# yuguangnudt/VEC_VAD

Hardware: AMD Instinct MI355X
Metric: spatio-temporal cubes/sec (train step) (higher is better)
Workload: dtype f32

## Files before the change

include/vecvad_hip.h:

```cpp
#ifndef VECVAD_HIP_H
#define VECVAD_HIP_H

#include <stddef.h>
#include <stdint.h>

#ifdef __cplusplus
extern "C" {
#endif

typedef void* vv_stream;

enum vv_status {
  VV_OK = 0,
  VV_ERR_BAD_ARG = 1,
  VV_ERR_LAUNCH = 2,
  VV_ERR_UNSUPPORTED = 3
};

enum vv_in_mode {
  VV_IN_PLAIN = 0,
  VV_IN_ACT = 1,
  VV_IN_POOL = 2,
  VV_IN_CAT = 3,
  VV_IN_CUBE = 4,
  VV_IN_BNBWD = 5
};

enum vv_conv_kind {
  VV_CONV3 = 0,
  VV_CONVT_FWD = 1,
  VV_CONVT_DGRAD = 2
};

typedef struct vv_view {
  float* ptr;
  int64_t gstride;
  int32_t cstride;
  int32_t coff;
} vv_view;

#define VV_CONV_BF16 1
#define VV_CONV_SRC_BF16 2
#define VV_CONV_OUT_BF16 8
#define VV_CONV_ALLSRC_BF16 16
#define VV_CONV_RELU 32
#define VV_CONV_NO_GEMM16 64
#define VV_CONV_NO_RING 128
typedef struct vv_conv_params {
  int32_t kind;
  int32_t in_mode;
  int32_t G, B;
  int32_t H, W;
  int32_t Cin;
  int32_t CinP;
  int32_t Cout;
  vv_view src0;
  const float* a;
  const float* b;
  int64_t ab_gstride;
  vv_view src1;
  int32_t csplit;
  int32_t pad0;
  const int32_t* chmap;
  const float* w;
  int64_t w_gstride;
  const float* bias;
  int64_t bias_gstride;
  vv_view out;
  float* stats;
  const float* bn_z; int64_t bn_z_gstride;
  const float* bn_a; const float* bn_b; const float* bn_mean; const float* bn_invstd; int64_t bn_gstride;
  float* bn_partial;
  vv_view out1;
  int32_t osplit;
  int32_t pad1;
} vv_conv_params;

int vv_conv_mfma(const vv_conv_params* p, vv_stream stream);
int vv_conv_ntiles(int32_t B, int32_t H, int32_t W);
int vv_conv_ntiles2(int32_t B, int32_t H, int32_t W, int32_t kind, int32_t flags);
int vv_convt_dgrad_ntiles(int32_t B, int32_t H, int32_t W, int32_t flags);

typedef struct vv_wgrad_params {
  int32_t kind;
  int32_t in_mode;
  int32_t G, B, H, W;
  int32_t Cin, CinP, Cout;
  int32_t ksplit;
  vv_view src0; const float* a; const float* b; int64_t ab_gstride;
  vv_view src1; int32_t csplit;
  int32_t pad0;
  const int32_t* chmap;
  vv_view dy;
  float* partial;
  int64_t partial_gstride;
  vv_view dy_z;
  const float* dy_bn; int64_t dy_bn_gstride;
} vv_wgrad_params;

int vv_wgrad_mfma(const vv_wgrad_params* p, vv_stream stream);
int vv_wgrad_ntiles(int32_t kind, int32_t B, int32_t H, int32_t W);

#define VV_WGRAD_X_BF16 2
#define VV_WGRAD_DY_BF16 1
int vv_wgrad_bf16(const vv_wgrad_params* p, vv_stream stream);
int vv_wgrad_bf16_plan(int32_t kind, int32_t B, int32_t H, int32_t W, int32_t CinP, int32_t Cout, int32_t* ntiles, int32_t* nblocks,
                       int32_t* kw);

int vv_wgrad_reduce(int32_t kind, int32_t G, int32_t Cin, int32_t CinP, int32_t Cout, int32_t nslab_per_tile,
                    const float* partial, int64_t partial_gstride, float* grad, int64_t grad_gstride,
                    vv_stream stream);
typedef struct vv_reduce_entry {
  int32_t kind, Cin, Cout, NCO, nslab, block_start;
  int64_t part_off, grad_off, grad_gstride;
} vv_reduce_entry;
int vv_wgrad_reduce_grouped(const vv_reduce_entry* table_dev, int32_t nentries, int32_t total_blocks, int32_t G, const float* partial,
                            int64_t partial_gstride, float* grads, vv_stream stream);

#define VV_PACK_BF16 4
typedef struct vv_pack_entry {
  int64_t src_off;
  int64_t dst_off;
  int32_t mode, K, KP, N;
} vv_pack_entry;
int vv_pack_weights(const vv_pack_entry* table_dev, int32_t nentries, int32_t G, const float* params,
                    int64_t params_gstride, float* packed, int64_t packed_gstride, int32_t max_elems,
                    vv_stream stream);

int vv_conv_wino(const vv_conv_params* p, vv_stream stream);
int vv_wino_ntiles(int32_t B, int32_t H);
// ... 285 lines not shown
```

vec_vad_amd/_lib.py:

```python
import ctypes as C
import os

import torch

HERE = os.path.dirname(os.path.abspath(__file__))
LIB_PATH = os.environ.get('VV_LIB_PATH') or os.path.join(HERE, 'csrc', 'libvecvad_hip.so')

c_i32, c_i64, c_f32, c_f64, c_vp = C.c_int32, C.c_int64, C.c_float, C.c_double, C.c_void_p

IN_PLAIN, IN_ACT, IN_POOL, IN_CAT, IN_CUBE, IN_BNBWD = 0, 1, 2, 3, 4, 5
BNBWD_TAB_ROWS = 7
CONV3, CONVT_FWD, CONVT_DGRAD = 0, 1, 2
CONV_BF16 = 1
CONV_SRC_BF16 = 2
PACK_BF16 = 4
BNBWD_DZ_BF16 = 1
BNBWD_PARTIALS_PER_CUBE = 2
BNBWD_DA_BF16 = 4
CONV_OUT_BF16 = 8
CONV_ALLSRC_BF16 = 16
CONV_RELU = 32
CONV_NO_GEMM16 = 64
CONV_NO_RING = 128
BNBWD_Y_BF16 = 8
BNBWD_PARTIALS_PER_TILE = 16
BNBWD_PARTIALS_PER_CTILE = 32
BNBWD_PARTIALS_PER_TILE44 = 64
BNBWD_PARTIALS_PER_TTILE = 128
WGRAD_X_BF16 = 2
WGRAD_DY_BF16 = 1


class View(C.Structure):
    _fields_ = [('ptr', c_vp), ('gstride', c_i64), ('cstride', c_i32), ('coff', c_i32)]


class ConvParams(C.Structure):
    _fields_ = [('kind', c_i32), ('in_mode', c_i32), ('G', c_i32), ('B', c_i32), ('H', c_i32), ('W', c_i32),
                ('Cin', c_i32), ('CinP', c_i32), ('Cout', c_i32),
                ('src0', View), ('a', c_vp), ('b', c_vp), ('ab_gstride', c_i64),
                ('src1', View), ('csplit', c_i32), ('pad0', c_i32), ('chmap', c_vp),
                ('w', c_vp), ('w_gstride', c_i64), ('bias', c_vp), ('bias_gstride', c_i64),
                ('out', View), ('stats', c_vp),
                ('bn_z', c_vp), ('bn_z_gstride', c_i64), ('bn_a', c_vp), ('bn_b', c_vp), ('bn_mean', c_vp), ('bn_invstd', c_vp),
                ('bn_gstride', c_i64), ('bn_partial', c_vp),
                ('out1', View), ('osplit', c_i32), ('pad1', c_i32)]


class WgradParams(C.Structure):
    _fields_ = [('kind', c_i32), ('in_mode', c_i32), ('G', c_i32), ('B', c_i32), ('H', c_i32), ('W', c_i32),
                ('Cin', c_i32), ('CinP', c_i32), ('Cout', c_i32), ('ksplit', c_i32),
                ('src0', View), ('a', c_vp), ('b', c_vp), ('ab_gstride', c_i64),
                ('src1', View), ('csplit', c_i32), ('pad0', c_i32), ('chmap', c_vp),
                ('dy', View), ('partial', c_vp), ('partial_gstride', c_i64),
                ('dy_z', View), ('dy_bn', c_vp), ('dy_bn_gstride', c_i64)]


class PackEntry(C.Structure):
    _fields_ = [('src_off', c_i64), ('dst_off', c_i64), ('mode', c_i32), ('K', c_i32), ('KP', c_i32), ('N', c_i32)]


class ReduceEntry(C.Structure):
    _fields_ = [('kind', c_i32), ('Cin', c_i32), ('Cout', c_i32), ('NCO', c_i32), ('nslab', c_i32), ('block_start', c_i32),
                ('part_off', c_i64), ('grad_off', c_i64), ('grad_gstride', c_i64)]


class FoldEntry(C.Structure):
    _fields_ = [('w_off', c_i64), ('b_off', c_i64), ('g_off', c_i64), ('beta_off', c_i64), ('rm_off', c_i64), ('rv_off', c_i64),
                ('cout', c_i32), ('row', c_i32)]


class BnBwdParams(C.Structure):
    _fields_ = [('G', c_i32), ('B', c_i32), ('H', c_i32), ('W', c_i32), ('C', c_i32), ('flags', c_i32),
                ('y', c_vp), ('y_gstride', c_i64),
                ('a', c_vp), ('b', c_vp), ('mean', c_vp), ('invstd', c_vp), ('ab_gstride', c_i64),
                ('dA', View), ('dpool', c_vp), ('dpool_gstride', c_i64),
                ('dz', c_vp), ('dz_gstride', c_i64), ('partial', c_vp)]


class OutconvParams(C.Structure):
    _fields_ = [('G', c_i32), ('B', c_i32), ('HW', c_i32), ('C', c_i32),
                ('y', c_vp), ('y_gstride', c_i64), ('a', c_vp), ('b', c_vp), ('ab_gstride', c_i64),
                ('w', c_vp), ('bias', c_vp), ('param_gstride', c_i64), ('oc', c_vp),
                ('tgt0', c_vp), ('tgt0_cstride', c_i32), ('pad0', c_i32),
                ('tgt1', c_vp), ('tgt1_cstride', c_i32), ('pad1', c_i32),
                ('tgt_src', c_vp), ('tgt_coff', c_vp), ('out4', c_vp), ('score', c_vp), ('gscale', c_vp),
                ('dout4', c_vp)]


class Conv2dParams(C.Structure):
    _fields_ = [('kind', c_i32), ('R', c_i32), ('stride', c_i32), ('B', c_i32), ('H', c_i32), ('W', c_i32),
                ('Cin', c_i32), ('CinP', c_i32), ('Cout', c_i32), ('CoutP', c_i32), ('src', View), ('w', c_vp),
                ('bias', c_vp), ('slope', c_f32), ('pad0', c_i32), ('out', View)]


_SIGS = {
    'vv_conv2d_mfma': (c_i32, [C.POINTER(Conv2dParams), c_vp]),
    'vv_conv2d_wino': (c_i32, [c_vp, c_i32, c_i32, c_i64, c_vp, c_vp, c_f32, c_vp, c_i32, c_i32, c_i32, c_i32, c_i32, c_i32, c_i32, c_vp]),
    'vv_conv2d_splitk_finish': (c_i32, [c_vp, c_i32, c_i64, c_i32, c_i32, c_vp, c_f32, c_vp, c_i32, c_i32, c_vp]),
    'vv_pack_conv2d': (c_i32, [c_vp, c_vp, c_i32, c_i32, c_i32, c_i32, c_i32, c_i32, c_vp]),
    'vv_conv3x3_n2': (c_i32, [c_vp, c_i32, c_i32, c_i32, c_i32, c_i32, c_vp, c_i32, c_vp, c_f32, c_vp, c_i32, c_i32, c_vp]),
    'vv_deconv4x4_c2': (c_i32, [c_vp, c_i32, c_i32, c_i32, c_i32, c_vp, c_vp, c_f32, c_vp, c_i32, c_i32, c_vp]),
    'vv_upsample4': (c_i32, [c_vp, c_vp, c_i32, c_i32, c_i32, c_i32, c_f32, c_vp]),
    'vv_conv_mfma': (c_i32, [C.POINTER(ConvParams), c_vp]),
    'vv_conv_wino': (c_i32, [C.POINTER(ConvParams), c_vp]),
    'vv_wino_ntiles': (c_i32, [c_i32, c_i32]),
# ... 153 lines not shown
```

vec_vad_amd/csrc/vv_conv.hip:

```cpp
#include "vv_common.h"
#ifndef VV_PD_BF
#define VV_PD_BF 1
#endif

namespace {

template <int KIND, int TH, int TW>
struct Geo {
  static constexpr int HH = KIND == VV_CONV3 ? TH + 2 : (KIND == VV_CONVT_FWD ? TH + 1 : 2 * TH + 1);
  static constexpr int HW = KIND == VV_CONV3 ? TW + 2 : (KIND == VV_CONVT_FWD ? TW + 1 : 2 * TW + 1);
  static constexpr int SP = KIND == VV_CONVT_DGRAD ? 2 : 1;
};

template <int TH, int TW, int NI, int NR, int KIND, int CK, bool BF, int S16, int MR>
__global__ void __launch_bounds__(VV_WG, (MR == 1 && BF) ? 4 : ((BF && KIND == VV_CONVT_DGRAD) ? 1 : ((NR == 1 && KIND != VV_CONVT_FWD && !(BF && NI >= 4)) ? 3 : 2)))
conv_mfma_kernel(const vv_conv_params p, const int NT, const int NN, const int total, const int nper) {
  using G_ = Geo<KIND, TH, TW>;
  constexpr int HH = G_::HH, HW = G_::HW, SP = G_::SP;
  static_assert(!BF || CK % 16 == 0, "bf16 K step = 16 channels");
  constexpr int S = BF ? CK / 2 + ((CK / 8) % 2 ? 8 : 4) : CK + 4;
  constexpr int S4 = S / 4;
  static_assert(S4 % 2 == 1, "odd float4 stride");
  static_assert(TH * TW * NI == 128 * MR, "tile pixels");
  constexpr int TN = NR * 32;
  constexpr int KGC = BF ? CK / 16 : CK / 8;
  constexpr int A4 = NI * HH * HW * S4;
  constexpr int BROWS = 9 * KGC * 2;
  constexpr int B4 = BROWS * TN;
  constexpr int NBT = (B4 + VV_WG - 1) / VV_WG;
  constexpr int ORS = TN + 8, OUT4 = (BF && KIND != VV_CONVT_FWD) ? (128 * MR * ORS * 2 + 15) / 16 : 0;
  constexpr int LDS4 = (A4 + B4) > OUT4 ? (A4 + B4) : OUT4;
  __shared__ float4 lds4[LDS4];
  float* lds = reinterpret_cast<float*>(lds4);
  const v4f* ldsA = reinterpret_cast<const v4f*>(lds4);
  const v4f* ldsB = reinterpret_cast<const v4f*>(lds4) + A4;

  int w = vv_xcd_remap(blockIdx.x, nper);
  if (w >= total) return;
  const int nn = w % NN; w /= NN;
  const int pt = w % NT; w /= NT;
  const int g = w;

  const int tid = threadIdx.x, lane = tid & 63, wave = tid >> 6, half = lane >> 5, l31 = lane & 31;
  const int H = p.H, W = p.W;
  const int tilesX = W / TW, tilesY = H / TH;
  const int tpi = tilesX * tilesY;
  const int img0 = (pt / tpi) * NI;
  const int trem = pt % tpi;
  const int ty0 = (trem / tilesX) * TH, tx0 = (trem % tilesX) * TW;

  const int SH = KIND == VV_CONVT_DGRAD ? 2 * H : H, SW = KIND == VV_CONVT_DGRAD ? 2 * W : W;
  const int oy0 = KIND == VV_CONV3 ? ty0 - 1 : (KIND == VV_CONVT_FWD ? ty0 : 2 * ty0 - 1);
  const int ox0 = KIND == VV_CONV3 ? tx0 - 1 : (KIND == VV_CONVT_FWD ? tx0 : 2 * tx0 - 1);

  const VVSrc s = vv_make_src(p, g, SH, SW);
  const int Cout = p.Cout, CinP = p.CinP, KQ = CinP >> 3;
  const int co0 = nn * TN;
  const float* __restrict__ wg = p.w + (int64_t)g * p.w_gstride;

  int abase[MR];
#pragma unroll
  for (int m = 0; m < MR; ++m) {
    const int pp = wave * (32 * MR) + m * 32 + l31;
    const int im = pp / (TH * TW), r = (pp / TW) % TH, c = pp % TW;
    abase[m] = ((im * HH + r * SP) * HW + c * SP) * S4 + half;
  }

  constexpr int NACC = KIND == VV_CONVT_FWD ? 4 : NR;
  static_assert(KIND != VV_CONVT_FWD || NR == 1, "transposed conv forward: 32-wide N tiles");
  v16f acc[MR][NACC];
#pragma unroll
  for (int m = 0; m < MR; ++m)
#pragma unroll
    for (int n = 0; n < NACC; ++n)
#pragma unroll
      for (int i = 0; i < 16; ++i) acc[m][n][i] = 0.f;

  constexpr bool BNF = BF && NR == 1 && KIND == VV_CONV3 && S16 == 3;
  static_assert(S16 != 3 || BNF, "S16 == 3: the 32-wide 3x3 launch with BatchNorm-backward sums");
  constexpr bool BNT = !BF && KIND == VV_CONVT_DGRAD && NR == 1 && MR == 1 && S16 == 4;
  static_assert(S16 != 4 || BNT, "S16 == 4: the fp32 stride-2 gather (128-pixel tiles, 32-wide N tiles) with BatchNorm-backward sums");
  float zt[BNT ? 16 : 1];
  if constexpr (BNT) {
    const float* zb = p.bn_z + (int64_t)g * p.bn_z_gstride + co0 + l31;
#pragma unroll
    for (int i = 0; i < 16; ++i) {
      const int row = (i & 3) + 8 * (i >> 2) + 4 * half;
      const int pp = wave * 32 + row;
      const int im = pp / (TH * TW), r = (pp / TW) % TH, c = pp % TW;
      zt[i] = img0 + im < p.B ? zb[((int64_t)((img0 + im) * H + ty0 + r) * W + tx0 + c) * Cout] : 0.f;
    }
  }
  constexpr int BN_QN = NR * 4, BN_NOUT = 128 * MR * BN_QN / VV_WG;
  const bool bnf = BNF && p.bn_partial != nullptr;
  uint4 zq[BNF ? BN_NOUT : 1];
  if constexpr (BNF) {
    if (bnf) {
      const unsigned short* zh = reinterpret_cast<const unsigned short*>(p.bn_z + (int64_t)g * p.bn_z_gstride) + co0 + (tid % BN_QN) * 8;
#pragma unroll
      for (int k = 0; k < BN_NOUT; ++k) {
        const int pp = (tid + k * VV_WG) / BN_QN;
        const int im = pp / (TH * TW), r = (pp / TW) % TH, c = pp % TW;
        zq[k] = img0 + im < p.B ? *reinterpret_cast<const uint4*>(zh + ((int64_t)((img0 + im) * H + ty0 + r) * W + tx0 + c) * Cout)
                                : make_uint4(0u, 0u, 0u, 0u);
      }
    }
  }

  VVStagerB<NI, HH, HW, S, ((BF && S16 >= 2) ? CK / 2 : CK)> stA;
  stA.init(s, ox0, tid);
  unsigned boff[NBT];
  float4 rb[NBT];
  const int KGT = BF ? (CinP >> 4) : KQ;
#pragma unroll
  for (int k = 0; k < NBT; ++k) {
    const int it = tid + k * VV_WG;
    const int col = it % TN, row = it / TN;
    const int hf = row & 1, tk = row >> 1;
    const int kg = tk % KGC, tap = tk / KGC;
    boff[k] = (B4 % VV_WG == 0 || it < B4) ? (unsigned)(((tap * KGT + kg) * 2 + hf) * Cout + co0 + col) * 16u : 0x80000000u;
  }
  const __amdgpu_buffer_rsrc_t rsW = __builtin_amdgcn_make_buffer_rsrc(const_cast<float*>(wg), 0, 0x7FFFFFFF, 0x00020000);
  auto issue = [&](const int c0) {
    if constexpr (BF && S16 >= 2) stA.prefetch16w(s, img0, oy0, ox0, c0, tid);
    else if constexpr (BF && S16 == 1) stA.prefetch16(s, img0, oy0, ox0, c0, tid);
    else stA.prefetch(s, img0, oy0, ox0, c0, tid);
    const int so = (BF ? (c0 >> 4) : (c0 >> 3)) * 2 * Cout * 16;
#pragma unroll
    for (int k = 0; k < NBT; ++k) {
      const v4f v = __builtin_amdgcn_raw_buffer_load_b128(rsW, boff[k], so, 0);
      rb[k] = make_float4(v.x, v.y, v.z, v.w);
    }
  };
  auto commit = [&]() {
    if constexpr (BF && S16 >= 2) stA.commit16w(lds, tid);
    else if constexpr (BF && S16 == 1) stA.commit_raw16(lds, tid);
    else if constexpr (BF) stA.commit_bf16(lds, tid);
    else stA.commit(lds, tid);
#pragma unroll
    for (int k = 0; k < NBT; ++k) {
      const int it = tid + k * VV_WG;
      if (B4 % VV_WG == 0 || it < B4) lds4[A4 + it] = rb[k];
    }
  };

  issue(0);
  for (int c0 = 0; c0 < CinP; c0 += CK) {
    if (c0) __syncthreads();
    commit();
    __syncthreads();
    if (c0 + CK < CinP) issue(c0 + CK);

    {
      constexpr int NIT = 9 * KGC;
      constexpr int PDW = VV_PD_BF;
      constexpr int PD = BF ? (NIT > PDW ? PDW : NIT - 1) : 1, RING = PD + 1;
      v4f fa[RING][MR], fb[RING][NR];
      auto rdA = [&](const int it, const int m) -> v4f {
        const int tap = it / KGC, kg = it % KGC;
        const int dy = KIND == VV_CONVT_FWD ? (tap / 3 == 0) : tap / 3, dx = KIND == VV_CONVT_FWD ? (tap % 3 == 0) : tap % 3;
        return ldsA[abase[m] + (dy * HW + dx) * S4 + kg * 2];
      };
      auto rdB = [&](const int it, const int n) -> v4f {
        const int tap = it / KGC, kg = it % KGC;
        return ldsB[((tap * KGC + kg) * 2 + half) * TN + n * 32 + l31];
      };
#pragma unroll
      for (int s = 0; s < PD; ++s) {
#pragma unroll
        for (int m = 0; m < MR; ++m) fa[s][m] = rdA(s, m);
#pragma unroll
        for (int n = 0; n < NR; ++n) fb[s][n] = rdB(s, n);
      }
      __builtin_amdgcn_sched_barrier(0);
#pragma unroll
      for (int it = 0; it < NIT; ++it) {
        const int cur = it % RING, nxt = (it + PD) % RING;
        int piece = 0;
        const int tapc = it / KGC;
        const int phc = ((tapc / 3 != 1) ? 2 : 0) + ((tapc % 3 != 1) ? 1 : 0);
#pragma unroll
        for (int m = 0; m < MR; ++m)
#pragma unroll
          for (int n = 0; n < NR; ++n) {
            const int an = KIND == VV_CONVT_FWD ? phc : n;
            if constexpr (BF) {
              acc[m][an] = __builtin_amdgcn_mfma_f32_32x32x16_bf16(__builtin_bit_cast(v8bf, fa[cur][m]),
                                                                   __builtin_bit_cast(v8bf, fb[cur][n]), acc[m][an], 0, 0, 0);
            } else {
              acc[m][an] = __builtin_amdgcn_mfma_f32_32x32x2f32(fa[cur][m].x, fb[cur][n].x, acc[m][an], 0, 0, 0);
              acc[m][an] = __builtin_amdgcn_mfma_f32_32x32x2f32(fa[cur][m].y, fb[cur][n].y, acc[m][an], 0, 0, 0);
              acc[m][an] = __builtin_amdgcn_mfma_f32_32x32x2f32(fa[cur][m].z, fb[cur][n].z, acc[m][an], 0, 0, 0);
              acc[m][an] = __builtin_amdgcn_mfma_f32_32x32x2f32(fa[cur][m].w, fb[cur][n].w, acc[m][an], 0, 0, 0);
            }
            if (it + PD < NIT) {
              const int last = (m == MR - 1 && n == NR - 1);
              do {
                if (piece < MR) fa[nxt][piece] = rdA(it + PD, piece);
                else if (piece < MR + NR) fb[nxt][piece - MR] = rdB(it + PD, piece - MR);
                ++piece;
              } while (last && piece < MR + NR);
            }
            __builtin_amdgcn_sched_barrier(0);
          }
      }
    }
  }

  const int OH = KIND == VV_CONVT_FWD ? 2 * H : H, OW = KIND == VV_CONVT_FWD ? 2 * W : W;
  float* __restrict__ outg = p.out.ptr + (int64_t)g * p.out.gstride + p.out.coff;
  const int ocs = p.out.cstride;
  const bool o16 = BF && (p.pad0 & VV_CONV_OUT_BF16);
  __bf16* __restrict__ outh = reinterpret_cast<__bf16*>(p.out.ptr + (int64_t)g * p.out.gstride) + p.out.coff;
  float bias[NR], s1[NR], s2[NR];
#pragma unroll
  for (int n = 0; n < NR; ++n) {
    bias[n] = p.bias ? p.bias[(int64_t)g * p.bias_gstride + co0 + n * 32 + l31] : 0.f;
    s1[n] = 0.f; s2[n] = 0.f;
  }
  const float relu_lo = (p.pad0 & VV_CONV_RELU) ? 0.f : -__builtin_inff();
  float bta = 0.f, btb = 0.f, bt1 = 0.f, bt2 = 0.f;
  bool tile_out = false;
  if constexpr (BF && KIND != VV_CONVT_FWD) tile_out = o16;
  if (tile_out) {
    if constexpr (BF && KIND != VV_CONVT_FWD) {
      constexpr int QN = TN / 8, NOUT = 128 * MR * QN / VV_WG;
      static_assert((128 * MR * QN) % VV_WG == 0 && VV_WG % QN == 0, "output items per thread, one channel group per thread");
      static_assert(!BNF || (QN == BN_QN && NOUT == BN_NOUT), "z items = output items");
      __syncthreads();
      unsigned short* lo = reinterpret_cast<unsigned short*>(lds4);
#pragma unroll
      for (int m = 0; m < MR; ++m)
#pragma unroll
        for (int i = 0; i < 16; ++i) {
          const int row = (i & 3) + 8 * (i >> 2) + 4 * half;
          const int pp = wave * (32 * MR) + m * 32 + row;
          const bool ok = img0 + pp / (TH * TW) < p.B;
#pragma unroll
          for (int n = 0; n < NR; ++n) {
            float v = acc[m][n][i] + bias[n];
            v = v < relu_lo ? relu_lo : v;
            const __bf16 hv = (__bf16)v;
            lo[pp * ORS + n * 32 + l31] = __builtin_bit_cast(unsigned short, hv);
            v = ok ? (float)hv : 0.f;
            s1[n] += v; s2[n] = fmaf(v, v, s2[n]);
          }
        }
      __syncthreads();
      __bf16* obase = outh + co0 + (tid % QN) * 8;
      if (p.out1.ptr && co0 + (tid % QN) * 8 >= p.osplit)
        obase = reinterpret_cast<__bf16*>(p.out1.ptr + (int64_t)g * p.out1.gstride) + p.out1.coff + (co0 + (tid % QN) * 8 - p.osplit);
      float bna[8], bnb[8], bnm[8], bni[8], bs1[8], bs2[8];
      if constexpr (BNF) {
        if (bnf) {
          const int64_t o = (int64_t)g * p.bn_gstride + co0 + (tid % QN) * 8;
#pragma unroll
          for (int j = 0; j < 8; ++j) { bna[j] = p.bn_a[o + j]; bnb[j] = p.bn_b[o + j]; bnm[j] = p.bn_mean[o + j]; bni[j] = p.bn_invstd[o + j]; bs1[j] = 0.f; bs2[j] = 0.f; }
        }
      }
#pragma unroll
      for (int k = 0; k < NOUT; ++k) {
        const int it = tid + k * VV_WG;
        const int pp = it / QN;
        const int im = pp / (TH * TW), r = (pp / TW) % TH, c = pp % TW;
        const int img = img0 + im;
        if (img < p.B) {
          const uint4 v = *reinterpret_cast<const uint4*>(lo + pp * ORS + (tid % QN) * 8);
          *reinterpret_cast<uint4*>(obase + ((int64_t)(img * OH + ty0 + r) * OW + tx0 + c) * ocs) = v;
          if constexpr (BNF) {
            if (bnf) {
              const unsigned dw[4] = {v.x, v.y, v.z, v.w}, zw[4] = {zq[k].x, zq[k].y, zq[k].z, zq[k].w};
#pragma unroll
              for (int j = 0; j < 4; ++j) {
                typedef float v2f_ __attribute__((ext_vector_type(2)));
                const v2f_ z2 = {__builtin_bit_cast(float, zw[j] << 16), __builtin_bit_cast(float, zw[j] & 0xFFFF0000u)};
                const v2f_ d2 = {__builtin_bit_cast(float, dw[j] << 16), __builtin_bit_cast(float, dw[j] & 0xFFFF0000u)};
                const v2f_ a2 = {bna[2 * j], bna[2 * j + 1]}, b2 = {bnb[2 * j], bnb[2 * j + 1]};
                const v2f_ on = __builtin_elementwise_fma(a2, z2, b2);
                const v2f_ dj = {on.x > 0.f ? d2.x : 0.f, on.y > 0.f ? d2.y : 0.f};
                v2f_ t1 = {bs1[2 * j], bs1[2 * j + 1]}, t2 = {bs2[2 * j], bs2[2 * j + 1]};
                t1 += dj;
                t2 = __builtin_elementwise_fma(dj, z2, t2);
                bs1[2 * j] = t1.x; bs1[2 * j + 1] = t1.y; bs2[2 * j] = t2.x; bs2[2 * j + 1] = t2.y;
              }
            }
          }
        }
      }
      if constexpr (BNF) {
        if (bnf) {
#pragma unroll
          for (int j = 0; j < 8; ++j) {
            static_assert(!BNF || QN == 4, "lanes with the same lane % 4");
            bs2[j] = bni[j] * (bs2[j] - bnm[j] * bs1[j]);
            bs1[j] += vv_dpp_ror<4>(bs1[j]); bs2[j] += vv_dpp_ror<4>(bs2[j]);
            bs1[j] += vv_dpp_ror<8>(bs1[j]); bs2[j] += vv_dpp_ror<8>(bs2[j]);
            bs1[j] += __shfl_xor(bs1[j], 16); bs2[j] += __shfl_xor(bs2[j], 16);
            bs1[j] += __shfl_xor(bs1[j], 32); bs2[j] += __shfl_xor(bs2[j], 32);
          }
          __syncthreads();
          if (lane < QN) {
#pragma unroll
            for (int j = 0; j < 8; ++j) { lds[wave * 2 * TN + lane * 8 + j] = bs1[j]; lds[wave * 2 * TN + TN + lane * 8 + j] = bs2[j]; }
          }
          __syncthreads();
          if (tid < 2 * TN) {
            const float t = (lds[tid] + lds[2 * TN + tid]) + (lds[4 * TN + tid] + lds[6 * TN + tid]);
            p.bn_partial[((int64_t)(g * NT + pt) * 2) * Cout + (tid / TN) * Cout + co0 + tid % TN] = t;
          }
        }
      }
    }
  } else {
  if constexpr (BNT) {
    const int64_t o = (int64_t)g * p.bn_gstride + co0 + l31;
    bta = p.bn_a[o]; btb = p.bn_b[o];
  }
#pragma unroll
  for (int m = 0; m < MR; ++m)
#pragma unroll
    for (int i = 0; i < 16; ++i) {
      const int row = (i & 3) + 8 * (i >> 2) + 4 * half;
      const int pp = wave * (32 * MR) + m * 32 + row;
      const int im = pp / (TH * TW), r = (pp / TW) % TH, c = pp % TW;
      const int img = img0 + im;
      if constexpr (BNT) {
        const float d = (img < p.B && fmaf(bta, zt[i], btb) > 0.f) ? acc[m][0][i] + bias[0] : 0.f;
        bt1 += d;
        bt2 = fmaf(d, zt[i], bt2);
      }
      if (img < p.B) {
        if constexpr (KIND == VV_CONVT_FWD) {
          const int64_t e = ((int64_t)(img * OH + 2 * (ty0 + r)) * OW + 2 * (tx0 + c)) * ocs + co0 + l31;
#pragma unroll
          for (int ph = 0; ph < 4; ++ph) {
            const float v = acc[m][ph][i] + bias[0];
            if (o16) outh[e + ((ph >> 1) * OW + (ph & 1)) * ocs] = (__bf16)v;
            else outg[e + ((ph >> 1) * OW + (ph & 1)) * ocs] = v;
          }
        } else {
          const int64_t e = ((int64_t)(img * OH + ty0 + r) * OW + tx0 + c) * ocs + co0 + l31;
#pragma unroll
          for (int n = 0; n < NR; ++n) {
            float v = acc[m][n][i] + bias[n];
            v = v < relu_lo ? relu_lo : v;
            if (o16) {
              const __bf16 hv = (__bf16)v;
              outh[e + n * 32] = hv;
              v = (float)hv;
            } else {
              outg[e + n * 32] = v;
            }
            s1[n] += v; s2[n] = fmaf(v, v, s2[n]);
          }
        }
      }
    }

  }
  if constexpr (BNT) {
    bt1 += __shfl_xor(bt1, 32);
    bt2 += __shfl_xor(bt2, 32);
    __syncthreads();
    if (half == 0) { lds[wave * 64 + l31] = bt1; lds[wave * 64 + 32 + l31] = bt2; }
    __syncthreads();
    if (tid < 32) {
      const float t1 = (lds[tid] + lds[64 + tid]) + (lds[128 + tid] + lds[192 + tid]);
      const float t2 = (lds[32 + tid] + lds[96 + tid]) + (lds[160 + tid] + lds[224 + tid]);
      const int64_t o = (int64_t)g * p.bn_gstride + co0 + tid;
      float* bp = p.bn_partial + ((int64_t)(g * NT + pt) * 2) * Cout + co0 + tid;
      bp[0] = t1;
      bp[Cout] = p.bn_invstd[o] * (t2 - p.bn_mean[o] * t1);
    }
  }
  if (p.stats) {
    __syncthreads();
#pragma unroll
    for (int n = 0; n < NR; ++n) {
      s1[n] += __shfl_xor(s1[n], 32);
      s2[n] += __shfl_xor(s2[n], 32);
      if (half == 0) {
        lds[(wave * NR + n) * 32 + l31] = s1[n];
        lds[4 * TN + (wave * NR + n) * 32 + l31] = s2[n];
      }
    }
    __syncthreads();
    if (tid < TN) {
      const int n = tid >> 5, l = tid & 31;
      float t1 = 0.f, t2 = 0.f;
#pragma unroll
      for (int wv = 0; wv < 4; ++wv) {
        t1 += lds[(wv * NR + n) * 32 + l];
        t2 += lds[4 * TN + (wv * NR + n) * 32 + l];
      }
      float* st = p.stats + ((int64_t)(g * NT + pt) * 2) * Cout + co0 + tid;
      st[0] = t1;
      st[Cout] = t2;
    }
  }
}

struct TileGeo { int TH, TW, NI; };
inline bool tile_geo(int H, int W, TileGeo* t) {
  if (H != W) return false;
  if (H == 32) { *t = {8, 32, 1}; return true; }
  if (H == 16) { *t = {16, 16, 1}; return true; }
  if (H == 8) { *t = {8, 8, 4}; return true; }
  if (H == 4) { *t = {4, 4, 16}; return true; }
  return false;
}

template <int TH, int TW, int NI, int NR, int KIND, int CK, bool BF = false, int S16 = 0, int MR = 2>
int launch(const vv_conv_params* p, hipStream_t st) {
  const int NT = ((p->B + NI - 1) / NI) * (p->H / TH) * (p->W / TW);
  const int NN = p->Cout / (NR * 32);
  const int total = p->G * NN * NT;
  const int nper = (total + 7) / 8;
  VV_LAUNCH((conv_mfma_kernel<TH, TW, NI, NR, KIND, CK, BF, S16, MR>), dim3(nper * 8), dim3(VV_WG), 0, st, *p, NT, NN,
                     total, nper);
  VV_CHECK_LAUNCH();
  return VV_OK;
}

template <int KIND, int CK, bool BF, int S16 = 0>
int dispatch(const vv_conv_params* p, hipStream_t st) {
  TileGeo t;
  if (!tile_geo(p->H, p->W, &t)) return VV_ERR_UNSUPPORTED;
  if constexpr (BF && KIND == VV_CONV3) {
    if (p->H == 16) return (p->Cout % 64) == 0 ? launch<8, 16, 1, 2, KIND, 16, BF, S16, 1>(p, st) : launch<8, 16, 1, 1, KIND, 16, BF, S16, 1>(p, st);
    if (p->H == 8) return (p->Cout % 64) == 0 ? launch<8, 8, 2, 2, KIND, 16, BF, S16, 1>(p, st) : launch<8, 8, 2, 1, KIND, 16, BF, S16, 1>(p, st);
    if (p->H == 4) return (p->Cout % 64) == 0 ? launch<4, 4, 8, 2, KIND, 16, BF, S16, 1>(p, st) : launch<4, 4, 8, 1, KIND, 16, BF, S16, 1>(p, st);
  }
  const int nt = ((p->B + t.NI - 1) / t.NI) * (p->H / t.TH) * (p->W / t.TW);
  const int64_t wide_min = (!BF && KIND == VV_CONVT_DGRAD) ? 512 : 1024;
  const bool wide = KIND != VV_CONVT_FWD && (p->Cout % 64) == 0 && (int64_t)p->G * nt * (p->Cout / 64) >= wide_min;
  constexpr int CKD = BF ? (KIND == VV_CONVT_DGRAD ? 16 : CK) : (KIND == VV_CONVT_DGRAD ? 8 : 16);
  constexpr int CK4 = BF ? 16 : 8;
  if constexpr (!BF && KIND != VV_CONV3) {
    if (p->H == 16 && KIND == VV_CONVT_DGRAD) return launch<8, 16, 1, 1, KIND, CKD, BF, S16, 1>(p, st);
    if (p->H == 8) return launch<8, 8, 2, 1, KIND, CKD, BF, S16, 1>(p, st);
    if (p->H == 4) return launch<4, 4, 8, 1, KIND, CK4, BF, S16, 1>(p, st);
  }
  if constexpr (KIND == VV_CONVT_FWD) {
    switch (p->H) {
      case 32: return launch<8, 32, 1, 1, KIND, CKD, BF, S16>(p, st);
      case 16: return launch<16, 16, 1, 1, KIND, CKD, BF, S16>(p, st);
      case 8: return launch<8, 8, 4, 1, KIND, CKD, BF, S16>(p, st);
      case 4: return launch<4, 4, 16, 1, KIND, CK4, BF, S16>(p, st);
    }
  } else {
    switch (p->H) {
      case 32: return wide ? launch<8, 32, 1, 2, KIND, CKD, BF, S16>(p, st) : launch<8, 32, 1, 1, KIND, CKD, BF, S16>(p, st);
      case 16: return wide ? launch<16, 16, 1, 2, KIND, CKD, BF, S16>(p, st) : launch<16, 16, 1, 1, KIND, CKD, BF, S16>(p, st);
      case 8: return wide ? launch<8, 8, 4, 2, KIND, CKD, BF, S16>(p, st) : launch<8, 8, 4, 1, KIND, CKD, BF, S16>(p, st);
      case 4: return wide ? launch<4, 4, 16, 2, KIND, CK4, BF, S16>(p, st) : launch<4, 4, 16, 1, KIND, CK4, BF, S16>(p, st);
    }
  }
  return VV_ERR_UNSUPPORTED;
}

}

extern "C" int vv_conv_ntiles(int32_t B, int32_t H, int32_t W) {
  TileGeo t;
  if (!tile_geo(H, W, &t)) return -1;
  return ((B + t.NI - 1) / t.NI) * (H / t.TH) * (W / t.TW);
}

extern "C" int vv_convt_dgrad_ntiles(int32_t B, int32_t H, int32_t W, int32_t flags) {
  if (H != W || (H != 16 && H != 8 && H != 4)) return -1;
  const int px = (flags & VV_CONV_BF16) ? 256 : 128;
  const int per_img = H * W;
  return per_img >= px ? B * (per_img / px) : (B + px / per_img - 1) / (px / per_img);
}

extern "C" int vv_conv_ntiles2(int32_t B, int32_t H, int32_t W, int32_t kind, int32_t flags) {
  if (vv_gemm16_flags(kind, flags)) return vv_conv_ntiles(B, H, W);
  if ((flags & VV_CONV_BF16) && kind == VV_CONV3 && H == W && H == 16) return B * 2;
  if ((flags & VV_CONV_BF16) && kind == VV_CONV3 && H == W && (H == 8 || H == 4)) return (B + (H == 8 ? 1 : 7)) / (H == 8 ? 2 : 8);
  if (!(flags & VV_CONV_BF16) && kind == VV_CONVT_DGRAD && H == W && (H == 16 || H == 8 || H == 4)) return vv_convt_dgrad_ntiles(B, H, W, 0);
  return vv_conv_ntiles(B, H, W);
}

extern "C" int vv_conv_mfma(const vv_conv_params* p, vv_stream stream) {
  if (!p || !p->src0.ptr || !p->w || !p->out.ptr) return VV_ERR_BAD_ARG;
  if (p->G <= 0 || p->B <= 0) return VV_ERR_BAD_ARG;
  if (p->Cout % 32) return VV_ERR_UNSUPPORTED;
  if (p->in_mode == VV_IN_BNBWD) return VV_ERR_UNSUPPORTED;
  hipStream_t st = (hipStream_t)stream;
  const bool bf = (p->pad0 & VV_CONV_BF16) != 0;
  if (bf && p->CinP % 16) return VV_ERR_BAD_ARG;
  if ((p->pad0 & VV_CONV_SRC_BF16) && !(bf && p->in_mode == VV_IN_PLAIN && p->kind != VV_CONVT_FWD && p->src0.coff % 2 == 0)) return VV_ERR_BAD_ARG;
  if ((p->pad0 & VV_CONV_OUT_BF16) && !bf) return VV_ERR_BAD_ARG;
  if ((p->pad0 & VV_CONV_OUT_BF16) && p->kind != VV_CONVT_FWD && (p->out.coff % 8 || p->out.cstride % 8)) return VV_ERR_BAD_ARG;
  if ((p->pad0 & VV_CONV_ALLSRC_BF16) && (!bf || p->in_mode == VV_IN_POOL || p->in_mode == VV_IN_CUBE)) return VV_ERR_BAD_ARG;
  if (p->CinP % 8) return VV_ERR_BAD_ARG;
  if (p->kind == VV_CONVT_FWD && p->stats) return VV_ERR_UNSUPPORTED;
  if (p->bn_partial && !bf && p->kind == VV_CONVT_DGRAD) {
    if (p->stats || p->out1.ptr || (p->H != 16 && p->H != 8 && p->H != 4) || p->H != p->W) return VV_ERR_UNSUPPORTED;
    if (!p->bn_z || !p->bn_a || !p->bn_b || !p->bn_mean || !p->bn_invstd) return VV_ERR_BAD_ARG;
  } else if (p->bn_partial) {
    if (!(bf && (p->pad0 & VV_CONV_OUT_BF16) && (p->pad0 & VV_CONV_ALLSRC_BF16) && p->kind == VV_CONV3)) return VV_ERR_UNSUPPORTED;
    if (p->H != 32 || p->W != 32 || p->Cout % 64 == 0 || p->stats || p->out1.ptr) return VV_ERR_UNSUPPORTED;
    if (!p->bn_z || !p->bn_a || !p->bn_b || !p->bn_mean || !p->bn_invstd) return VV_ERR_BAD_ARG;
  }
  if (p->out1.ptr) {
    if (!(bf && (p->pad0 & VV_CONV_OUT_BF16) && p->kind == VV_CONV3)) return VV_ERR_UNSUPPORTED;
    if (p->osplit <= 0 || p->osplit >= p->Cout || p->osplit % 32 || p->out1.cstride != p->out.cstride ||
        p->out1.gstride != p->out.gstride || p->out1.coff % 8)
      return VV_ERR_BAD_ARG;
  }
  const int sm = !bf ? 0 : ((p->pad0 & VV_CONV_ALLSRC_BF16) ? 2 : ((p->pad0 & VV_CONV_SRC_BF16) ? 1 : 0));
  if (vv_gemm16_flags(p->kind, p->pad0) && p->H <= 16) return vv_conv_gemm16(p, st);
  if (sm == 2 && vv_conv_ring16_ok(p)) return vv_conv_ring16(p, st);
  switch (p->kind) {
    case VV_CONV3:
      if (p->CinP % 16) return VV_ERR_BAD_ARG;
      if (sm == 2 && p->bn_partial) return launch<8, 32, 1, 1, VV_CONV3, 16, true, 3>(p, st);
      if (sm == 2) return dispatch<VV_CONV3, 16, true, 2>(p, st);
      if (sm == 1) return dispatch<VV_CONV3, 16, true, 1>(p, st);
      return bf ? dispatch<VV_CONV3, 16, true>(p, st) : dispatch<VV_CONV3, 16, false>(p, st);
    case VV_CONVT_FWD:
      if (p->CinP % 16) return VV_ERR_BAD_ARG;
      if (sm == 2) return dispatch<VV_CONVT_FWD, 16, true, 2>(p, st);
      return bf ? dispatch<VV_CONVT_FWD, 16, true>(p, st) : dispatch<VV_CONVT_FWD, 16, false>(p, st);
    case VV_CONVT_DGRAD:
      if (bf && p->CinP % 16) return VV_ERR_BAD_ARG;
      if (!bf && p->bn_partial) {
        if (p->H == 16) return launch<8, 16, 1, 1, VV_CONVT_DGRAD, 8, false, 4, 1>(p, st);
        if (p->H == 8) return launch<8, 8, 2, 1, VV_CONVT_DGRAD, 8, false, 4, 1>(p, st);
        return launch<4, 4, 8, 1, VV_CONVT_DGRAD, 8, false, 4, 1>(p, st);
      }
      if (sm == 2) return dispatch<VV_CONVT_DGRAD, 8, true, 2>(p, st);
      if (sm == 1) return dispatch<VV_CONVT_DGRAD, 8, true, 1>(p, st);
      return bf ? dispatch<VV_CONVT_DGRAD, 8, true>(p, st) : dispatch<VV_CONVT_DGRAD, 8, false>(p, st);
  }
  return VV_ERR_BAD_ARG;
}
```

Measured before the change: 29000.

## Use 64-wide output-channel tiles for fp32 transposed-conv forward and dgrad kernels

Adds NR=2 (64-wide N) variants of the fp32 transposed-conv forward and stride-2 dgrad MFMA kernels on the 128-pixel tiles, including the BatchNorm-backward fused path. Each workgroup now computes twice the output channels per staged input tile, so input reuse goes up and fewer workgroups are launched. A heuristic based on CU count and workgroups per CU picks the wide path, with env and flag overrides. The cost is more accumulator registers and lower occupancy, a forced plain input mode on the wide dgrad path, and 32-bit buffer-offset limits.

```diff
diff --git a/include/vecvad_hip.h b/include/vecvad_hip.h
--- a/include/vecvad_hip.h
+++ b/include/vecvad_hip.h
@@ -46,6 +46,8 @@
 #define VV_CONV_RELU 32
 #define VV_CONV_NO_GEMM16 64
 #define VV_CONV_NO_RING 128
+#define VV_CONV_CONVT_NARROW 256
+#define VV_CONV_CONVT_WIDE 512
 typedef struct vv_conv_params {
   int32_t kind;
   int32_t in_mode;
diff --git a/vec_vad_amd/_lib.py b/vec_vad_amd/_lib.py
--- a/vec_vad_amd/_lib.py
+++ b/vec_vad_amd/_lib.py
@@ -22,6 +22,8 @@
 CONV_RELU = 32
 CONV_NO_GEMM16 = 64
 CONV_NO_RING = 128
+CONV_CONVT_NARROW = 256
+CONV_CONVT_WIDE = 512
 BNBWD_Y_BF16 = 8
 BNBWD_PARTIALS_PER_TILE = 16
 BNBWD_PARTIALS_PER_CTILE = 32
diff --git a/vec_vad_amd/csrc/vv_conv.hip b/vec_vad_amd/csrc/vv_conv.hip
--- a/vec_vad_amd/csrc/vv_conv.hip
+++ b/vec_vad_amd/csrc/vv_conv.hip
@@ -1,6 +1,10 @@
 #include "vv_common.h"
 #ifndef VV_PD_BF
 #define VV_PD_BF 1
+#endif
+
+#ifndef VV_CONVT_WIDE_WGS
+#define VV_CONVT_WIDE_WGS 3
 #endif
 
 namespace {
@@ -13,7 +17,7 @@
 };
 
 template <int TH, int TW, int NI, int NR, int KIND, int CK, bool BF, int S16, int MR>
-__global__ void __launch_bounds__(VV_WG, (MR == 1 && BF) ? 4 : ((BF && KIND == VV_CONVT_DGRAD) ? 1 : ((NR == 1 && KIND != VV_CONVT_FWD && !(BF && NI >= 4)) ? 3 : 2)))
+__global__ void __launch_bounds__(VV_WG, (MR == 1 && BF) ? 4 : ((BF && KIND == VV_CONVT_DGRAD) ? 1 : ((!BF && KIND == VV_CONVT_DGRAD && MR == 1 && NR == 2) ? VV_CONVT_WIDE_WGS : ((NR == 1 && KIND != VV_CONVT_FWD && !(BF && NI >= 4)) ? 3 : 2))))
 conv_mfma_kernel(const vv_conv_params p, const int NT, const int NN, const int total, const int nper) {
   using G_ = Geo<KIND, TH, TW>;
   constexpr int HH = G_::HH, HW = G_::HW, SP = G_::SP;
@@ -53,7 +57,10 @@
   const int oy0 = KIND == VV_CONV3 ? ty0 - 1 : (KIND == VV_CONVT_FWD ? ty0 : 2 * ty0 - 1);
   const int ox0 = KIND == VV_CONV3 ? tx0 - 1 : (KIND == VV_CONVT_FWD ? tx0 : 2 * tx0 - 1);
 
-  const VVSrc s = vv_make_src(p, g, SH, SW);
+  VVSrc s_ = vv_make_src(p, g, SH, SW);
+  if constexpr (!BF && KIND == VV_CONVT_DGRAD && NR == 2 && MR == 1) s_.mode = VV_IN_PLAIN;
+  const VVSrc s = s_;
+  if constexpr (!BF && KIND == VV_CONVT_FWD && NR == 2) __builtin_assume(s.mode != VV_IN_POOL && s.mode != VV_IN_CUBE);
   const int Cout = p.Cout, CinP = p.CinP, KQ = CinP >> 3;
   const int co0 = nn * TN;
   const float* __restrict__ wg = p.w + (int64_t)g * p.w_gstride;
@@ -66,8 +73,8 @@
     abase[m] = ((im * HH + r * SP) * HW + c * SP) * S4 + half;
   }
 
-  constexpr int NACC = KIND == VV_CONVT_FWD ? 4 : NR;
-  static_assert(KIND != VV_CONVT_FWD || NR == 1, "transposed conv forward: 32-wide N tiles");
+  constexpr int NACC = KIND == VV_CONVT_FWD ? 4 * NR : NR;
+  static_assert(KIND != VV_CONVT_FWD || NR == 1 || (NR == 2 && MR == 1 && !BF), "transposed conv forward: 32-wide N tiles, 64-wide on the fp32 128-pixel tiles");
   v16f acc[MR][NACC];
 #pragma unroll
   for (int m = 0; m < MR; ++m)
@@ -78,18 +85,29 @@
 
   constexpr bool BNF = BF && NR == 1 && KIND == VV_CONV3 && S16 == 3;
   static_assert(S16 != 3 || BNF, "S16 == 3: the 32-wide 3x3 launch with BatchNorm-backward sums");
-  constexpr bool BNT = !BF && KIND == VV_CONVT_DGRAD && NR == 1 && MR == 1 && S16 == 4;
-  static_assert(S16 != 4 || BNT, "S16 == 4: the fp32 stride-2 gather (128-pixel tiles, 32-wide N tiles) with BatchNorm-backward sums");
-  float zt[BNT ? 16 : 1];
-  if constexpr (BNT) {
-    const float* zb = p.bn_z + (int64_t)g * p.bn_z_gstride + co0 + l31;
+  constexpr bool BNT = !BF && KIND == VV_CONVT_DGRAD && NR <= 2 && MR == 1 && S16 == 4;
+  static_assert(S16 != 4 || BNT, "S16 == 4: the fp32 stride-2 gather (128-pixel tiles, 32- or 64-wide N tiles) with BatchNorm-backward sums");
+  float zt[BNT ? NR : 1][BNT ? 16 : 1];
+  auto request_z = [&](const int n) {
+    if constexpr (!BNT) return;
+    const float* zb = p.bn_z + (int64_t)g * p.bn_z_gstride + co0 + n * 32 + l31;
+    const __amdgpu_buffer_rsrc_t rsZ = __builtin_amdgcn_make_buffer_rsrc(const_cast<float*>(p.bn_z + (int64_t)g * p.bn_z_gstride), 0, 0x7FFFFFFF, 0x00020000);
 #pragma unroll
     for (int i = 0; i < 16; ++i) {
       const int row = (i & 3) + 8 * (i >> 2) + 4 * half;
       const int pp = wave * 32 + row;
       const int im = pp / (TH * TW), r = (pp / TW) % TH, c = pp % TW;
-      zt[i] = img0 + im < p.B ? zb[((int64_t)((img0 + im) * H + ty0 + r) * W + tx0 + c) * Cout] : 0.f;
-    }
+      if constexpr (NR > 1) {
+        const unsigned off = img0 + im < p.B ? (unsigned)((((img0 + im) * H + ty0 + r) * W + tx0 + c) * Cout + co0 + l31) * 4u : 0x80000000u;
+        zt[n][i] = __builtin_bit_cast(float, __builtin_amdgcn_raw_buffer_load_b32(rsZ, off + (unsigned)n * 128u, 0, 0));
+      } else {
+        zt[n][i] = img0 + im < p.B ? zb[((int64_t)((img0 + im) * H + ty0 + r) * W + tx0 + c) * Cout] : 0.f;
+      }
+    }
+  };
+  if constexpr (BNT) {
+#pragma unroll
+    for (int n = 0; n < NR; ++n) request_z(n);
   }
   constexpr int BN_QN = NR * 4, BN_NOUT = 128 * MR * BN_QN / VV_WG;
   const bool bnf = BNF && p.bn_partial != nullptr;
@@ -112,6 +130,7 @@
   unsigned boff[NBT];
   float4 rb[NBT];
   const int KGT = BF ? (CinP >> 4) : KQ;
+  constexpr bool BLIN = !BF && KIND == VV_CONVT_FWD && NR == 2 && VV_WG == 2 * KGC * TN;
 #pragma unroll
   for (int k = 0; k < NBT; ++k) {
     const int it = tid + k * VV_WG;
@@ -128,7 +147,8 @@
     const int so = (BF ? (c0 >> 4) : (c0 >> 3)) * 2 * Cout * 16;
 #pragma unroll
     for (int k = 0; k < NBT; ++k) {
-      const v4f v = __builtin_amdgcn_raw_buffer_load_b128(rsW, boff[k], so, 0);
+      const v4f v = BLIN ? __builtin_amdgcn_raw_buffer_load_b128(rsW, boff[0], so + k * KGT * 2 * Cout * 16, 0)
+                         : __builtin_amdgcn_raw_buffer_load_b128(rsW, boff[k], so, 0);
       rb[k] = make_float4(v.x, v.y, v.z, v.w);
     }
   };
@@ -183,7 +203,7 @@
         for (int m = 0; m < MR; ++m)
 #pragma unroll
           for (int n = 0; n < NR; ++n) {
-            const int an = KIND == VV_CONVT_FWD ? phc : n;
+            const int an = KIND == VV_CONVT_FWD ? phc * NR + n : n;
             if constexpr (BF) {
               acc[m][an] = __builtin_amdgcn_mfma_f32_32x32x16_bf16(__builtin_bit_cast(v8bf, fa[cur][m]),
                                                                    __builtin_bit_cast(v8bf, fb[cur][n]), acc[m][an], 0, 0, 0);
@@ -219,7 +239,9 @@
     s1[n] = 0.f; s2[n] = 0.f;
   }
   const float relu_lo = (p.pad0 & VV_CONV_RELU) ? 0.f : -__builtin_inff();
-  float bta = 0.f, btb = 0.f, bt1 = 0.f, bt2 = 0.f;
+  float bta[NR], btb[NR], bt1[NR], bt2[NR];
+#pragma unroll
+  for (int n = 0; n < NR; ++n) { bta[n] = 0.f; btb[n] = 0.f; bt1[n] = 0.f; bt2[n] = 0.f; }
   bool tile_out = false;
   if constexpr (BF && KIND != VV_CONVT_FWD) tile_out = o16;
   if (tile_out) {
@@ -314,7 +336,8 @@
   } else {
   if constexpr (BNT) {
     const int64_t o = (int64_t)g * p.bn_gstride + co0 + l31;
-    bta = p.bn_a[o]; btb = p.bn_b[o];
+#pragma unroll
+    for (int n = 0; n < NR; ++n) { bta[n] = p.bn_a[o + n * 32]; btb[n] = p.bn_b[o + n * 32]; }
   }
 #pragma unroll
   for (int m = 0; m < MR; ++m)
@@ -325,19 +348,24 @@
       const int im = pp / (TH * TW), r = (pp / TW) % TH, c = pp % TW;
       const int img = img0 + im;
       if constexpr (BNT) {
-        const float d = (img < p.B && fmaf(bta, zt[i], btb) > 0.f) ? acc[m][0][i] + bias[0] : 0.f;
-        bt1 += d;
-        bt2 = fmaf(d, zt[i], bt2);
+#pragma unroll
+        for (int n = 0; n < NR; ++n) {
+          const float d = (img < p.B && fmaf(bta[n], zt[n][i], btb[n]) > 0.f) ? acc[m][n][i] + bias[n] : 0.f;
+          bt1[n] += d;
+          bt2[n] = fmaf(d, zt[n][i], bt2[n]);
+        }
       }
       if (img < p.B) {
         if constexpr (KIND == VV_CONVT_FWD) {
           const int64_t e = ((int64_t)(img * OH + 2 * (ty0 + r)) * OW + 2 * (tx0 + c)) * ocs + co0 + l31;
 #pragma unroll
-          for (int ph = 0; ph < 4; ++ph) {
-            const float v = acc[m][ph][i] + bias[0];
-            if (o16) outh[e + ((ph >> 1) * OW + (ph & 1)) * ocs] = (__bf16)v;
-            else outg[e + ((ph >> 1) * OW + (ph & 1)) * ocs] = v;
-          }
+          for (int n = 0; n < NR; ++n)
+#pragma unroll
+            for (int ph = 0; ph < 4; ++ph) {
+              const float v = acc[m][ph * NR + n][i] + bias[n];
+              if (o16) outh[e + ((ph >> 1) * OW + (ph & 1)) * ocs + n * 32] = (__bf16)v;
+              else outg[e + ((ph >> 1) * OW + (ph & 1)) * ocs + n * 32] = v;
+            }
         } else {
           const int64_t e = ((int64_t)(img * OH + ty0 + r) * OW + tx0 + c) * ocs + co0 + l31;
 #pragma unroll
@@ -359,14 +387,17 @@
 
   }
   if constexpr (BNT) {
-    bt1 += __shfl_xor(bt1, 32);
-    bt2 += __shfl_xor(bt2, 32);
     __syncthreads();
-    if (half == 0) { lds[wave * 64 + l31] = bt1; lds[wave * 64 + 32 + l31] = bt2; }
+#pragma unroll
+    for (int n = 0; n < NR; ++n) {
+      bt1[n] += __shfl_xor(bt1[n], 32);
+      bt2[n] += __shfl_xor(bt2[n], 32);
+      if (half == 0) { lds[wave * 2 * TN + n * 32 + l31] = bt1[n]; lds[wave * 2 * TN + TN + n * 32 + l31] = bt2[n]; }
+    }
     __syncthreads();
-    if (tid < 32) {
-      const float t1 = (lds[tid] + lds[64 + tid]) + (lds[128 + tid] + lds[192 + tid]);
-      const float t2 = (lds[32 + tid] + lds[96 + tid]) + (lds[160 + tid] + lds[224 + tid]);
+    if (tid < TN) {
+      const float t1 = (lds[tid] + lds[2 * TN + tid]) + (lds[4 * TN + tid] + lds[6 * TN + tid]);
+      const float t2 = (lds[TN + tid] + lds[3 * TN + tid]) + (lds[5 * TN + tid] + lds[7 * TN + tid]);
       const int64_t o = (int64_t)g * p.bn_gstride + co0 + tid;
       float* bp = p.bn_partial + ((int64_t)(g * NT + pt) * 2) * Cout + co0 + tid;
       bp[0] = t1;
@@ -422,6 +453,15 @@
   return VV_OK;
 }
 
+inline bool convt_wide(const vv_conv_params* p, int nt, int wgs_per_cu) {
+  if ((p->Cout % 64) || (p->pad0 & VV_CONV_CONVT_NARROW) || p->in_mode == VV_IN_POOL || p->in_mode == VV_IN_CUBE) return false;
+  if (p->kind == VV_CONVT_DGRAD && p->in_mode != VV_IN_PLAIN) return false;
+  if (p->pad0 & VV_CONV_CONVT_WIDE) return true;
+  static const int mode = [] { const char* e = getenv("VV_CONVT_WIDE"); return (e && e[0] == '0') ? 0 : ((e && e[0] == '2') ? 2 : 1); }();
+  const int64_t rounds = p->kind == VV_CONVT_FWD ? 4 : 1;
+  return mode == 2 || (mode == 1 && (int64_t)p->G * nt * (p->Cout / 64) >= rounds * vv_num_cus() * wgs_per_cu);
+}
+
 template <int KIND, int CK, bool BF, int S16 = 0>
 int dispatch(const vv_conv_params* p, hipStream_t st) {
   TileGeo t;
@@ -437,9 +477,12 @@
   constexpr int CKD = BF ? (KIND == VV_CONVT_DGRAD ? 16 : CK) : (KIND == VV_CONVT_DGRAD ? 8 : 16);
   constexpr int CK4 = BF ? 16 : 8;
   if constexpr (!BF && KIND != VV_CONV3) {
-    if (p->H == 16 && KIND == VV_CONVT_DGRAD) return launch<8, 16, 1, 1, KIND, CKD, BF, S16, 1>(p, st);
-    if (p->H == 8) return launch<8, 8, 2, 1, KIND, CKD, BF, S16, 1>(p, st);
-    if (p->H == 4) return launch<4, 4, 8, 1, KIND, CK4, BF, S16, 1>(p, st);
+    const bool w128 = (p->H == 16 || p->H == 8 || p->H == 4) &&
+                      convt_wide(p, vv_convt_dgrad_ntiles(p->B, p->H, p->W, 0), KIND == VV_CONVT_FWD ? 2 : VV_CONVT_WIDE_WGS);
+    if constexpr (KIND == VV_CONVT_DGRAD)
+      if (p->H == 16) return w128 ? launch<8, 16, 1, 2, KIND, CKD, BF, S16, 1>(p, st) : launch<8, 16, 1, 1, KIND, CKD, BF, S16, 1>(p, st);
+    if (p->H == 8) return w128 ? launch<8, 8, 2, 2, KIND, CKD, BF, S16, 1>(p, st) : launch<8, 8, 2, 1, KIND, CKD, BF, S16, 1>(p, st);
+    if (p->H == 4) return w128 ? launch<4, 4, 8, 2, KIND, CK4, BF, S16, 1>(p, st) : launch<4, 4, 8, 1, KIND, CK4, BF, S16, 1>(p, st);
   }
   if constexpr (KIND == VV_CONVT_FWD) {
     switch (p->H) {
@@ -527,9 +570,10 @@
     case VV_CONVT_DGRAD:
       if (bf && p->CinP % 16) return VV_ERR_BAD_ARG;
       if (!bf && p->bn_partial) {
-        if (p->H == 16) return launch<8, 16, 1, 1, VV_CONVT_DGRAD, 8, false, 4, 1>(p, st);
-        if (p->H == 8) return launch<8, 8, 2, 1, VV_CONVT_DGRAD, 8, false, 4, 1>(p, st);
-        return launch<4, 4, 8, 1, VV_CONVT_DGRAD, 8, false, 4, 1>(p, st);
+        const bool w128 = convt_wide(p, vv_convt_dgrad_ntiles(p->B, p->H, p->W, 0), VV_CONVT_WIDE_WGS) && (int64_t)p->B * p->H * p->W * p->Cout * 4 < 0x7FFFFFFF;
+        if (p->H == 16) return w128 ? launch<8, 16, 1, 2, VV_CONVT_DGRAD, 8, false, 4, 1>(p, st) : launch<8, 16, 1, 1, VV_CONVT_DGRAD, 8, false, 4, 1>(p, st);
+        if (p->H == 8) return w128 ? launch<8, 8, 2, 2, VV_CONVT_DGRAD, 8, false, 4, 1>(p, st) : launch<8, 8, 2, 1, VV_CONVT_DGRAD, 8, false, 4, 1>(p, st);
+        return w128 ? launch<4, 4, 8, 2, VV_CONVT_DGRAD, 8, false, 4, 1>(p, st) : launch<4, 4, 8, 1, VV_CONVT_DGRAD, 8, false, 4, 1>(p, st);
       }
       if (sm == 2) return dispatch<VV_CONVT_DGRAD, 8, true, 2>(p, st);
       if (sm == 1) return dispatch<VV_CONVT_DGRAD, 8, true, 1>(p, st);
```

Result: faster. 29330, median of 6 (+1.1%).
